# lmfaber/karma

Hardware: AMD Instinct MI355X
Metric: contigs+reads/sec for k-mer vec + shared-read graph build; HBM GB/s vs roofline (higher is better)
Workload: dtype u32 keys / i64 counts / f64 div

## Files before the change

### include/karma.h

```cpp
#ifndef KARMA_H
#define KARMA_H

#include <stddef.h>
#include <stdint.h>

#ifdef __cplusplus
extern "C" {
#endif

#define KARMA_OK 0
#define KARMA_ERR_ARG (-1)
#define KARMA_ERR_KMER (-2)
#define KARMA_ERR_HIP (-3)
#define KARMA_ERR_OOM (-4)
#define KARMA_ERR_ZERO_DIV (-5)
#define KARMA_ERR_UNSORTED (-6)
#define KARMA_ERR_STATE (-7)
#define KARMA_ERR_PARSE (-8)
#define KARMA_ERR_COMM (-9)
#define KARMA_ERR_STALL (-10)

#define KARMA_KMER_5P6 (-1)

int karma_version(void);
// ... 82 lines not shown

int karma_knn_rows(karma_ctx* ctx, const double* x, int64_t n, int64_t m, int64_t ld, int x_is_device,
                   int64_t row_lo, int64_t row_hi, int k, int32_t* idx, double* dist, int out_is_device);
int karma_knn_tile(int* query_rows, int* cand_rows, int* col_panel, int* k_max);

int karma_knn_block(karma_ctx* ctx, const double* q, int64_t nq, int64_t ldq, int q_is_device,
                    const double* c, int64_t nc, int64_t ldc, int c_is_device,
                    int64_t m, int64_t cand_base, int k,
                    uint64_t* keys, int32_t* idx, int state_is_device,
                    int first, int cand_split);
int karma_knn_merge(karma_ctx* ctx, uint64_t* keys, int32_t* idx,
                    const uint64_t* keys_b, const int32_t* idx_b,
                    int64_t nq, int k, int state_is_device);
int karma_knn_finish(karma_ctx* ctx, const uint64_t* keys, const int32_t* idx, int64_t nq, int k, int state_is_device,
                     int32_t* out_idx, double* out_dist, int out_is_device);
int karma_knn_block_split(karma_ctx* ctx, int64_t nq, int64_t nc, int cand_split, int* used);

typedef struct karma_pairs karma_pairs;
#define KARMA_REC_SORTED 0
#define KARMA_REC_UNSORTED 1
#define KARMA_REC_FLAGGED 2
int karma_graph_records(karma_ctx* ctx, const uint32_t* records, int64_t n_records, int64_t n_contigs, int flags,
                        int is_device, karma_pairs** out);
typedef struct karma_graph_job karma_graph_job;
int karma_graph_records_begin(karma_ctx* ctx, const uint32_t* records, int64_t n_records, int64_t n_contigs,
                              int flags, int is_device, karma_graph_job** job);
int karma_graph_records_end(karma_graph_job* job, karma_pairs** out);
int karma_graph_split_hint(karma_ctx* ctx, const int64_t* bounds, int nranks);
int karma_records_flag(karma_ctx* ctx, const uint32_t* records, int64_t n_records, int rec_format, int is_device,
                       uint32_t* out, int out_is_device, int64_t* n_reads);
int karma_records_flag_tile(int* per_thread, int* per_wave, int* per_block);
int karma_classify_launches(uint64_t* pairs, uint64_t* flagged);
int karma_graph_classify_occupancy(karma_ctx* ctx, int64_t n_contigs, int rec_format, int* blocks_per_cu);
int karma_graph_eq(karma_ctx* ctx, const int64_t* cls_off, const uint32_t* members, const int64_t* counts,
                   const uint8_t* pair_skip, int64_t n_classes, int64_t n_contigs, int is_device, karma_pairs** out);
int karma_graph_eq_compact(karma_ctx* ctx, const uint8_t* sizes, const uint32_t* members, int64_t n_members,
                           const uint32_t* counts, int64_t C, int64_t n_contigs, karma_pairs** out);
int karma_pairs_merge(karma_ctx* ctx, const uint64_t* keys, const int64_t* counts, int64_t n, int is_device,
                      karma_pairs** out);
int karma_pairs_merge_runs(karma_ctx* ctx, const uint64_t* keys, const int64_t* counts, const int64_t* run_off,
                           int n_runs, int is_device, karma_pairs** out);
int karma_merge_tile(int* tile, int* lds_keys, int* max_runs, int* search_group);
int karma_step_tail_tile(karma_ctx* ctx, int* v, int n);
int karma_pairs_get_kc(karma_pairs* p, int64_t* kc_dev);
int karma_pairs_merge_runs_kc(karma_ctx* ctx, const int64_t* kc_dev, const int64_t* run_off, int n_runs,
                              karma_pairs** out);
int karma_pairs_destroy(karma_pairs* p);
int karma_pairs_rebind(karma_pairs* p, karma_ctx* ctx);
int karma_pairs_count(karma_pairs* p, int64_t* n);
int karma_pairs_device(karma_pairs* p, const uint64_t** keys, const int64_t** counts);
int karma_pairs_get(karma_pairs* p, uint64_t* keys, int64_t* counts, uint64_t* first, int is_device);
int karma_pairs_split(karma_pairs* p, const int64_t* bounds, int nranks, int64_t* starts);
int karma_pairs_split_kc(karma_pairs* p, const int64_t* bounds, int nranks, int64_t* starts, int64_t* kc_dev);
int karma_pairs_totals(karma_pairs* p, int64_t* totals_dev, int64_t n_contigs);

typedef struct karma_edges karma_edges;
#define KARMA_MODE_READS 0
#define KARMA_MODE_EQ 1
int karma_edges_from_pairs(karma_ctx* ctx, karma_pairs* p, int mode, const int64_t* totals_dev, int64_t n_contigs,
                           karma_edges** out, int64_t* n_edges);
int karma_edges_begin(karma_ctx* ctx, karma_pairs* p, int mode, int64_t n_contigs, karma_edges** out,
                      int64_t** totals_dev);
int karma_edges_end(karma_edges* e, int64_t* n_edges);
int karma_edges_count(karma_edges* e, int64_t* n_edges);
int karma_edges_destroy(karma_edges* e);
int karma_edges_get(karma_edges* e, uint32_t* a, uint32_t* b, int64_t* shared, double* weight, uint64_t* first,
                    int is_device);
int karma_edges_totals(karma_edges* e, int64_t* totals, int is_device);
int karma_edges_get_all(karma_edges* e, uint32_t* a, uint32_t* b, int64_t* s, double* w, uint64_t* first,
                        int64_t* totals, int is_device);
int karma_edges_get_ordered(karma_edges* e, uint32_t* a, uint32_t* b, double* w, int is_device);

typedef struct karma_step karma_step;
#define KARMA_STEP_KEEP 1
#define KARMA_STEP_SEQUENTIAL 2
#define KARMA_STEP_FLAGGED 8
// ... 79 lines not shown
```

### karma_amd/_lib.py

```python

from __future__ import annotations

import ctypes
import os
import types
import weakref

import numpy as np

HERE = os.path.dirname(os.path.abspath(__file__))
LIB_PATH = os.environ.get("KARMA_LIB") or os.path.join(HERE, "libkarma_hip.so")

KARMA_OK = 0
KARMA_ERR_ARG = -1
KARMA_ERR_KMER = -2
KARMA_ERR_HIP = -3
KARMA_ERR_OOM = -4
KARMA_ERR_ZERO_DIV = -5
KARMA_ERR_UNSORTED = -6
KARMA_ERR_STATE = -7
KARMA_ERR_PARSE = -8
KARMA_ERR_COMM = -9
KARMA_ERR_STALL = -10

# ... 58 lines not shown
    "karma_contigs_destroy": [_c_p],
    "karma_contigs_info": [_c_p, _I64P, _I64P, _I64P, _I64P],
    "karma_kmer_plan_create": [_c_p, _c_p, _i32, _PP],
    "karma_kmer_plan_destroy": [_c_p],
    "karma_kmer_presence_words": [_c_p, _I64P],
    "karma_kmer_presence_get": [_c_p, _c_p],
    "karma_kmer_presence_set": [_c_p, _c_p],
    "karma_kmer_presence_merge": [_c_p, _c_p, _i32],
    "karma_kmer_exceptions_count": [_c_p, _I64P],
    "karma_kmer_exceptions_get": [_c_p, _c_p],
    "karma_kmer_exceptions_set": [_c_p, _c_p, _i64],
    "karma_kmer_plan_finalize": [_c_p, _I64P],
    "karma_kmer_plan_finalize_async": [_c_p],
    "karma_kmer_plan_finalize_wait": [_c_p, _I64P],
    "karma_kmer_columns": [_c_p, _c_p],
    "karma_kmer_profile": [_c_p, _c_p, _i64, _i32],
    "karma_kmer_profile_rows": [_c_p, _i64, _i64, _c_p, _i64, _i32],
    "karma_kmer_profile_side": [_c_p, _c_p, _i64, _c_p],
    "karma_ctx_join": [_c_p, _c_p],
    "karma_ctx_set_side_headroom": [_c_p, _i32],
    "karma_kmer_row_totals": [_c_p, _c_p],
    "karma_knn_rows": [_c_p, _c_p, _i64, _i64, _i64, _i32, _i64, _i64, _i32, _c_p, _c_p, _i32],
    "karma_knn_tile": [ctypes.POINTER(ctypes.c_int)] * 4,
    "karma_knn_block": [_c_p, _c_p, _i64, _i64, _i32, _c_p, _i64, _i64, _i32, _i64, _i64, _i32, _c_p, _c_p, _i32, _i32,
                        _i32],
    "karma_knn_merge": [_c_p, _c_p, _c_p, _c_p, _c_p, _i64, _i32, _i32],
    "karma_knn_finish": [_c_p, _c_p, _c_p, _i64, _i32, _i32, _c_p, _c_p, _i32],
    "karma_knn_block_split": [_c_p, _i64, _i64, _i32, ctypes.POINTER(ctypes.c_int)],
    "karma_graph_records": [_c_p, _c_p, _i64, _i64, _i32, _i32, _PP],
    "karma_graph_records_begin": [_c_p, _c_p, _i64, _i64, _i32, _i32, _PP],
    "karma_graph_records_end": [_c_p, _PP],
    "karma_graph_split_hint": [_c_p, _c_p, _i32],
    "karma_graph_classify_occupancy": [_c_p, _i64, _i32, ctypes.POINTER(ctypes.c_int)],
    "karma_records_flag": [_c_p, _c_p, _i64, _i32, _i32, _c_p, _i32, _I64P],
    "karma_records_flag_tile": [ctypes.POINTER(ctypes.c_int)] * 3,
    "karma_classify_launches": [_c_p, _c_p],
    "karma_graph_eq": [_c_p, _c_p, _c_p, _c_p, _c_p, _i64, _i64, _i32, _PP],
    "karma_graph_eq_compact": [_c_p, _c_p, _c_p, _i64, _c_p, _i64, _i64, _PP],
    "karma_pairs_merge": [_c_p, _c_p, _c_p, _i64, _i32, _PP],
    "karma_pairs_merge_runs": [_c_p, _c_p, _c_p, _c_p, _i32, _i32, _PP],
    "karma_pairs_merge_runs_kc": [_c_p, _c_p, _c_p, _i32, _PP],
    "karma_merge_tile": [ctypes.POINTER(ctypes.c_int)] * 4,
    "karma_pairs_get_kc": [_c_p, _c_p],
    "karma_pairs_destroy": [_c_p],
    "karma_pairs_rebind": [_c_p, _c_p],
    "karma_pairs_count": [_c_p, _I64P],
    "karma_pairs_device": [_c_p, _PP, _PP],
    "karma_pairs_get": [_c_p, _c_p, _c_p, _c_p, _i32],
    "karma_pairs_split": [_c_p, _c_p, _i32, _c_p],
    "karma_pairs_totals": [_c_p, _c_p, _i64],
    "karma_edges_from_pairs": [_c_p, _c_p, _i32, _c_p, _i64, _PP, _I64P],
    "karma_edges_begin": [_c_p, _c_p, _i32, _i64, _PP, _PP],
    "karma_edges_end": [_c_p, _I64P],
    "karma_edges_count": [_c_p, _I64P],
    "karma_pairs_split_kc": [_c_p, _c_p, _i32, _c_p, _c_p],
    "karma_edges_destroy": [_c_p],
    "karma_edges_get": [_c_p, _c_p, _c_p, _c_p, _c_p, _c_p, _i32],
    "karma_edges_totals": [_c_p, _c_p, _i32],
    "karma_edges_get_all": [_c_p, _c_p, _c_p, _c_p, _c_p, _c_p, _c_p, _i32],
    "karma_edges_get_ordered": [_c_p, _c_p, _c_p, _c_p, _i32],
    "karma_api_calls": [_c_p],
    "karma_step_create": [_c_p, _c_p, _c_p, _i32, _i64, _c_p, _i32, _i32, _PP],
    "karma_step_run": [_c_p, _c_p, _c_p, _i64, _i32, _c_p],
    "karma_step_sync": [_c_p],
    "karma_step_info": [_c_p, _c_p, _i32],
    "karma_step_profile": [_c_p, _PP, _I64P, _I64P],
    "karma_step_columns": [_c_p, _c_p],
    "karma_step_edges": [_c_p, _PP],
    "karma_step_newest_edges": [_c_p, _c_p, _c_p, _c_p, _c_p, _c_p, _i64, _i32, _I64P, _c_p],
    "karma_step_destroy": [_c_p],
    "karma_step_tail_tile": [_c_p, _c_p, _i32],
    "karma_synth_contig_lengths": [_u64, _i64, _i32, _i32, _c_p],
    "karma_synth_contig_bases": [_u64, _c_p, _i64, _i32, _c_p],
    "karma_synth_n_genes": [_u64, _i64, _i32, _I64P],
    "karma_synth_genes": [_u64, _i64, _i32, _c_p, _c_p],
    "karma_synth_read_counts": [_u64, _c_p, _c_p, _i64, _i64, _i64, _i32, _c_p],
    "karma_synth_read_records": [_u64, _c_p, _c_p, _i64, _i64, _i64, _i32, _c_p, _c_p],
    "karma_synth_eq_classes": [_u64, _c_p, _c_p, _i64, _i64, _i64, _i32, _I64P, _I64P, _c_p, _c_p, _c_p],
    "karma_fasta_parse": [_c_p, ctypes.c_size_t, _i32, _PP],
    "karma_fasta_info": [_c_p, _I64P, _I64P, _I64P, ctypes.POINTER(ctypes.c_int)],
    "karma_fasta_get": [_c_p, _c_p, _c_p, _c_p, _c_p, _c_p],
    "karma_fasta_view": [_c_p, _PP, _PP, _PP, _PP, _PP],
    "karma_fasta_destroy": [_c_p],
    "karma_eq_parse": [_c_p, ctypes.c_size_t, _i32, _PP],
    "karma_eq_info": [_c_p, _I64P, _I64P, _I64P, _I64P],
    "karma_eq_get": [_c_p, _c_p, _c_p, _c_p, _c_p, _c_p, _c_p],
    "karma_eq_get_compact": [_c_p, _c_p, _c_p, _c_p, _c_p, _c_p],
    "karma_eq_destroy": [_c_p],
    "karma_sam_parse": [_c_p, ctypes.c_size_t, _i32, _i32, _PP],
    "karma_sam_info": [_c_p, _I64P, _I64P, _I64P, _I64P, _I64P],
    "karma_sam_get": [_c_p, _c_p, _c_p, _c_p, _c_p, _c_p],
    "karma_sam_destroy": [_c_p],
    "karma_adj_from_edges": [_c_p, _i64, _c_p, _c_p, _c_p, _c_p, _i64, _i32, _PP],
    "karma_adj_from_lists": [_c_p, _i64, _c_p, _c_p, _c_p, _c_p, _i32, _PP],
    "karma_adj_view": [_c_p, _c_p, _i64, _PP],
    "karma_adj_keep": [_c_p, _c_p, _i64, _PP],
    "karma_adj_view_summary": [_c_p, _c_p, _i64, _c_p, _c_p, _i32, _c_p, _c_p, _c_p, _i64, _I64P,
                               ctypes.POINTER(ctypes.c_int)],
    "karma_adj_node_stats": [_c_p, _c_p, _c_p],
    "karma_adj_info": [_c_p, _I64P, _I64P],
    "karma_adj_get": [_c_p, _c_p, _c_p, _c_p, _c_p],
    "karma_adj_degrees": [_c_p, _c_p],
    "karma_adj_node_weights": [_c_p, _c_p],
    "karma_adj_edge_list": [_c_p, _c_p, _c_p, _i64, _i32, _c_p, _i64, _I64P],
# ... 250 lines not shown

def flag_tile():
    v = [ctypes.c_int(0) for _ in range(3)]
    call("karma_records_flag_tile", *[ctypes.byref(x) for x in v])
    return tuple(x.value for x in v)


def knn_tile():
    v = [ctypes.c_int(0) for _ in range(4)]
    call("karma_knn_tile", *[ctypes.byref(x) for x in v])
    return tuple(x.value for x in v)


def knn_block_split(ctx, nq, nc, cand_split=0):
    used = ctypes.c_int(0)
    call("karma_knn_block_split", ctx.h if ctx is not None else None, int(nq), int(nc), int(cand_split),
         ctypes.byref(used))
    return used.value


def merge_tile():
    v = [ctypes.c_int(0) for _ in range(4)]
    call("karma_merge_tile", *[ctypes.byref(x) for x in v])
    return tuple(x.value for x in v)


def step_tail_tile(ctx=None):
    v = np.zeros(8, np.int32)
    call("karma_step_tail_tile", ctx.h if ctx is not None else None, ptr(v), 8)
    return types.SimpleNamespace(MT=int(v[0]), MLDS=int(v[1]), MFAST=int(v[2]), MG=int(v[3]), ET=int(v[4]),
                                 MAX_RUNS=int(v[5]), merge_blocks=int(v[6]), edge_blocks=int(v[7]))


def dtype_code(dtype):
    return _DTYPE_CODE[np.dtype(dtype)]


_DEFAULT_CTX = {}


def default_context(device=0):
    ctx = _DEFAULT_CTX.get(device)
    if ctx is None:
        ctx = _DEFAULT_CTX[device] = Context(device)
    return ctx
```

### karma_amd/csrc/graph_sets.hip

```cpp

#include <algorithm>
#include <cstdlib>
#include <cstring>
#include <memory>
#include <type_traits>

#include "karma_internal.h"
#include "sets_ctrl.h"

using namespace karma;

namespace {

#include "graph_device.h"

typedef unsigned int u32x4 __attribute__((ext_vector_type(4)));

constexpr int kMaxB = 2048;
constexpr int kMaxBc = 512;
constexpr int kNarrowB = 512, kNarrowBc = 128;
constexpr int kCrSmax = 64;
constexpr int kCrPieces = 512;
constexpr int kCgShift = 18;
constexpr int kOneGroupB = 128;
// ... 1294 lines not shown
                wslot[lane] = -1;
                wave_lds_order();
                if (len && excl >= w0 && excl < w0 + 64u) wslot[excl - w0] = lane;
                wave_lds_order();
                const int rr = wave_max_incl(max(wslot[lane], carry));
                carry = __builtin_amdgcn_readlane(rr, 63);
                const int64_t off = (int64_t)(((uint64_t)(uint32_t)__shfl((int)((uint64_t)roff >> 32), rr) << 32) |
                                              (uint32_t)__shfl((int)(uint32_t)roff, rr));
                if (j < Tn) e[u] = data[off + j];
            }
#pragma unroll
            for (int u = 0; u < kWin; ++u)
                if (j0 + 64u * u + lane < Tn) count(e[u]);
        }
        if (pipe) {
            if (r0 + threads >= r_hi) break;
        } else if (__syncthreads_or(stop != nullptr && *stop != 0)) {
            return;
        }
    }
}

__device__ __forceinline__ void group_range(const unsigned* n_flush, int n_groups, int grp, int64_t* f_lo,
                                            int64_t* f_hi) {
    const int64_t nf = *n_flush;
    const int64_t per = (nf + n_groups - 1) / n_groups;
    *f_lo = min(nf, grp * per);
    *f_hi = min(nf, *f_lo + per);
}

constexpr int kCRT = 1024;
constexpr int kHistMax = 1 << (kMaxBwCompact + 2 + 3);

__global__ void __launch_bounds__(kCRT) code_reduce_kernel(const uint16_t* __restrict__ cent, RunDir dir, int Bc,
                                                           int bwc, int n_cg, uint32_t* __restrict__ part_ch) {
    __shared__ uint32_t h[kHistMax];
    __shared__ int slots[kCRT];
    const int bucket = blockIdx.x / n_cg, grp = blockIdx.x % n_cg;
    const int hn = 1 << (bwc + 3);
    for (int i = threadIdx.x; i < hn; i += kCRT) h[i] = 0;
    __syncthreads();
    int64_t f_lo, f_hi;
    group_range(dir.n, n_cg, grp, &f_lo, &f_hi);
    const int64_t R = f_hi - f_lo;
    const int S = R > 0 ? (int)max<int64_t>(1, min<int64_t>(kCrSmax, (kCrPieces + R - 1) / R)) : 1;
    auto slot = [](uint32_t c) { return c ^ ((c >> 5) & 31u); };
    auto add = [&](uint32_t c) {
        if (c != CodeStream::kPadV)
            __hip_atomic_fetch_add(&h[slot(c)], 1u, __ATOMIC_RELAXED, __HIP_MEMORY_SCOPE_WORKGROUP);
    };
    stream_runs(
        reinterpret_cast<const u32x4*>(cent), f_lo * S, f_hi * S, kCRT,
        [&](int64_t v, int64_t* beg, uint32_t* len) {
            const int64_t f = v / S;
            const uint32_t s = (uint32_t)(v - f * S);
            const uint32_t* o = dir.off + f * (Bc + 1) + bucket;
            const uint32_t L = (o[1] - o[0]) >> 3, seg = (L + S - 1) / S;
            const uint32_t lo = min(L, s * seg), hi = min(L, lo + seg);
            *beg = ((dir.base[f] + o[0]) >> 3) + lo;
            *len = hi - lo;
        },
        [&](const u32x4 v) {
            add(v.x & 0xFFFFu), add(v.x >> 16), add(v.y & 0xFFFFu), add(v.y >> 16);
            add(v.z & 0xFFFFu), add(v.z >> 16), add(v.w & 0xFFFFu), add(v.w >> 16);
        },
        nullptr, slots);
    __syncthreads();
    uint32_t* out = part_ch + (int64_t)blockIdx.x * hn;
    for (int i = threadIdx.x; i < hn; i += kCRT) out[i] = h[slot(i)];
}

__device__ __forceinline__ uint32_t nibble_sum(uint32_t x) {
    x = (x & 0x0F0F0F0Fu) + ((x >> 4) & 0x0F0F0F0Fu);
    return (x * 0x01010101u) >> 24;
}
constexpr int kBackList = 2048;
__global__ void __launch_bounds__(kCRT) code_seg_reduce_kernel(const uint16_t* __restrict__ segs,
                                                               const uint4* __restrict__ hdr,
                                                               const uint8_t* __restrict__ dir, int64_t n_chunks,
                                                               uint32_t seg_cap, int dir_cap, int bwc, int n_cg,
                                                               uint32_t* __restrict__ part_ch, uint32_t list_cap,
                                                               int slotted) {
    __shared__ uint32_t h[kHistMax];
    __shared__ int slots[kCRT];
    __shared__ uint32_t blist[kBackList];
    __shared__ uint32_t nlist;
    const int bucket = blockIdx.x / n_cg, grp = blockIdx.x % n_cg;
    const int hn = 1 << (bwc + 3);
    for (int i = threadIdx.x; i < hn; i += kCRT) h[i] = 0;
    if (threadIdx.x == 0) nlist = 0;
    __syncthreads();
    const int64_t per = (n_chunks + n_cg - 1) / n_cg;
    const int64_t c_lo = min(n_chunks, (int64_t)grp * per), c_hi = min(n_chunks, c_lo + per);
    const int wave = __builtin_amdgcn_readfirstlane(threadIdx.x >> 6), lane = threadIdx.x & 63;
    auto slot = [](uint32_t c) { return c ^ ((c >> 5) & 31u); };
    auto add = [&](uint32_t c) {
        if (c != 0xFFFFu) __hip_atomic_fetch_add(&h[slot(c)], 1u, __ATOMIC_RELAXED, __HIP_MEMORY_SCOPE_WORKGROUP);
    };
    auto add8 = [&](const u32x4 v) {
        add(v.x & 0xFFFFu), add(v.x >> 16), add(v.y & 0xFFFFu), add(v.y >> 16);
        add(v.z & 0xFFFFu), add(v.z >> 16), add(v.w & 0xFFFFu), add(v.w >> 16);
    };
    const int bw_ = bucket >> 3, bs = 4 * (bucket & 7);
    auto list_back = [&](int64_t c, uint32_t bmw) {
        if ((bmw >> (bucket & 31)) & 1u) {
            const uint32_t i = __hip_atomic_fetch_add(&nlist, 1u, __ATOMIC_RELAXED, __HIP_MEMORY_SCOPE_WORKGROUP);
            if (i < list_cap) blist[i] = (uint32_t)(c - c_lo);
        }
    };
    if (slotted) {
        const uint32_t* const hw = reinterpret_cast<const uint32_t*>(hdr + 2) + (bucket < 32 ? 0 : 1);
        const uint32_t loff = (uint32_t)(lane >> 3) * seg_cap * (kBinQ * 2) + 16u * (lane & 7);
        const uint32_t tstr = 8u * seg_cap * (kBinQ * 2);
        auto load = [&](u32x4 (&v)[8], uint32_t& bm, int64_t c0, auto whole) {
            const char* const p = reinterpret_cast<const char*>(segs + (c0 * seg_cap + bucket) * kBinQ);
#pragma unroll
            for (int t = 0; t < 8; ++t)
                if (whole || c0 + 8 * t + (lane >> 3) < c_hi)
                    v[t] = *reinterpret_cast<const u32x4*>(p + (loff + t * tstr));
            if (whole || c0 + lane < c_hi) bm = hw[4 * kBinHdr * (c0 + lane)];
        };
        auto count = [&](const u32x4 (&v)[8], uint32_t bm, int64_t c0, auto whole) {
// ... 78 lines not shown
        uint64_t mb = lanes((bm >> bucket) & 1ull);
        if (!mb) continue;
        const uint32_t nb = h1.w;
        const uint32_t d[4] = {h2.z, h2.w, h3.x, h3.y};
        uint32_t hit = 0;
#pragma unroll
        for (int k = 0; k < 16; ++k)
            hit |= (((d[k >> 2] >> (8 * (k & 3))) & 0xFFu) == bb && (uint32_t)k < nb) ? 1u << k : 0u;
        for (uint32_t base = 0;;) {
            for (;;) {
                const uint64_t mm = lanes(in_mask(mb) && hit != 0u);
                if (!mm) break;
                uint32_t sg = 0;
                if (hit) {
                    const uint32_t k = (uint32_t)__builtin_ctz(hit);
                    hit &= hit - 1u;
                    sg = (uint32_t)c * seg_cap + seg_cap - 1u - (base + k);
                }
                stream8(mm, sg);
            }
            base += 16;
            mb &= lanes(base < nb);
            if (!mb) break;
            if (in_mask(mb)) {
                const u32x4 q = *reinterpret_cast<const u32x4*>(dir + c * (int64_t)dir_cap + base);
                const uint32_t e[4] = {q.x, q.y, q.z, q.w};
#pragma unroll
                for (int k = 0; k < 16; ++k)
                    hit |= (((e[k >> 2] >> (8 * (k & 3))) & 0xFFu) == bb && base + k < nb) ? 1u << k : 0u;
            }
        }
    }
    __syncthreads();
    uint32_t* out = part_ch + (int64_t)blockIdx.x * hn;
    for (int i = threadIdx.x; i < hn; i += kCRT) out[i] = h[slot(i)];
}

constexpr int kRT = 1024;
constexpr int kBand = 8192;
constexpr int kHashR = 4096;
constexpr int kHashF = 8192;
constexpr int kFT = 512;
constexpr int kSlotCap = kBand + kHashF;

template <int CAP, int THREADS>
struct HTab {
    uint32_t* keys;
    uint32_t* vals;
    int* nuniq;
    __device__ void init() {
        for (int t = threadIdx.x; t < CAP; t += THREADS) {
            keys[t] = kEmpty;
            vals[t] = 0;
        }
        if (threadIdx.x == 0) *nuniq = 0;
    }
    __device__ __forceinline__ bool insert(uint32_t key, uint32_t c) {
        uint32_t h = hash32(key) & (CAP - 1);
        for (int probe = 0; probe < CAP; ++probe) {
            const uint32_t k = __hip_atomic_load(&keys[h], __ATOMIC_RELAXED, __HIP_MEMORY_SCOPE_WORKGROUP);
            if (k == key) {
                atomicAdd(&vals[h], c);
                return true;
            }
            if (k == kEmpty) {
                const uint32_t old = atomicCAS(&keys[h], kEmpty, key);
                if (old == kEmpty || old == key) {
                    if (old == kEmpty) atomicAdd(nuniq, 1);
// ... 1165 lines not shown

void sets_release(SetsJob* job) {
    if (!job) return;
    job->ctx->job_open = false;
    job->ctx->mark_set = false;
    delete job;
}

int records_to_pairs_sets(karma_ctx* ctx, RecIn rec, int64_t A, int64_t N, karma_pairs* out) {
    if (N > kMaxCompactN) return records_to_pairs_wide(ctx, rec, A, N, out);
    SetsJob* job = nullptr;
    KARMA_TRY(sets_begin(ctx, rec, A, N, SetsOpts{}, &job));
    return sets_end(job, out);
}

}

extern "C" int karma_graph_classify_occupancy(karma_ctx* ctx, int64_t n_contigs, int rec_format,
                                              int* blocks_per_cu) {
    using namespace karma;
    KARMA_CHECK(ctx && blocks_per_cu && n_contigs >= 1 && n_contigs <= kMaxCompactN, KARMA_ERR_ARG,
                "karma_graph_classify_occupancy: bad arguments (n_contigs %lld)", (long long)n_contigs);
    KARMA_TRY(ctx_begin(ctx));
    Geo g{};
    KARMA_TRY(make_geo(n_contigs, &g));
    const bool bin = class_binned(g.Bc);
    const size_t lds = bin ? class_bin_lds(g.Bc) : 0;
    return with_classify(rec_format == KARMA_REC_FLAGGED, g.Bc >= kAppendMinBc, bin, false, [&](auto kern) -> int {
        KARMA_HIP(hipOccupancyMaxActiveBlocksPerMultiprocessor(blocks_per_cu, reinterpret_cast<const void*>(kern),
                                                               kCW, lds));
        return KARMA_OK;
    });
}
```

### karma_amd/csrc/step.hip

```cpp
#include <algorithm>
#include <chrono>
#include <cstdlib>
#include <cstring>
#include <deque>
#include <initializer_list>
#include <memory>
#include <thread>
#include <vector>

#include "karma_internal.h"
#include "sets_ctrl.h"
#include "step_schedule.h"

using namespace karma;

namespace {

constexpr int kRing = 64;
constexpr int kLag = 3;

enum StepErr : int64_t { kErrOrder = 1, kErrRange = 2, kErrPartition = 4, kErrZeroTotal = 8, kErrMergeOrder = 16 };
struct StepStatus {
    uint64_t seq;
    int64_t slow;
    int64_t err;
    int64_t U;
    int64_t E;
    int64_t pad[3];
};
static_assert(sizeof(StepStatus) == 64, "status entry");

constexpr int kET = 512;
constexpr int kMaxRuns = 64;

__device__ __forceinline__ bool is_head(const uint64_t* __restrict__ k, int64_t i, uint64_t key) {
    return i == 0 || k[i - 1] != key;
}
__device__ __forceinline__ int64_t run_sum(const uint64_t* __restrict__ k, const int64_t* __restrict__ c, int64_t n,
                                           int64_t i, uint64_t key) {
    int64_t s = c[i];
    for (int64_t j = i + 1; j < n && k[j] == key; ++j) s += c[j];
    return s;
}

__global__ void __launch_bounds__(kET) step_edge_count_kernel(const uint64_t* __restrict__ keys,
                                                              const int64_t* __restrict__ counts,
                                                              const int64_t* __restrict__ n_dev, int64_t n_tot,
                                                              int64_t* __restrict__ totals,
                                                              int64_t* __restrict__ tile_cnt,
                                                              int64_t* __restrict__ st) {
    const int64_t n = *n_dev;
    if (blockIdx.x == 0 && threadIdx.x < 3) st[threadIdx.x] = 0;
    const int64_t stride = (int64_t)gridDim.x * kET, gid = (int64_t)blockIdx.x * kET + threadIdx.x;
    const int64_t a_first = n ? (int64_t)(keys[0] >> 32) : n_tot;
    const int64_t a_last = n ? (int64_t)(keys[n - 1] >> 32) : n_tot;
    for (int64_t c = gid; c < min(a_first, n_tot); c += stride) totals[c] = 0;
    for (int64_t c = a_last + 1 + gid; c < n_tot; c += stride) totals[c] = 0;
    const int64_t tiles = (n + kET - 1) / kET;
    for (int64_t t = blockIdx.x; t < tiles; t += gridDim.x) {
        const int64_t i = t * kET + threadIdx.x;
        bool f = false;
        if (i < n) {
            const uint64_t k = keys[i];
            const uint32_t a = (uint32_t)(k >> 32), b = (uint32_t)k;
            if (i > 0) {
                const uint32_t pa = (uint32_t)(keys[i - 1] >> 32);
                const uint32_t lim = (int64_t)a < n_tot ? a : (uint32_t)n_tot;
                for (uint32_t c = pa + 1; c < lim; ++c) totals[c] = 0;
                if ((int64_t)a < n_tot && pa != a && a != b) totals[a] = 0;
            } else if ((int64_t)a < n_tot && a != b) {
                totals[a] = 0;
            }
            if (is_head(keys, i, k) && (int64_t)b < n_tot) {
                const int64_t s = run_sum(keys, counts, n, i, k);
                if (a == b) totals[a] = s;
                else f = s != 0;
            }
        }
        const int cnt = __syncthreads_count(f);
        if (threadIdx.x == 0) tile_cnt[t] = cnt;
    }
}

__global__ void __launch_bounds__(kET) step_edge_write_kernel(
    const uint64_t* __restrict__ keys, const int64_t* __restrict__ counts, const int64_t* __restrict__ n_dev,
    const int64_t* __restrict__ totals, const int64_t* __restrict__ tile_cnt, uint32_t* __restrict__ ea,
    uint32_t* __restrict__ eb, int64_t* __restrict__ es, double* __restrict__ ew, int64_t* __restrict__ st,
    int64_t n_tot) {
    __shared__ int64_t wsum[kET / 64];
    __shared__ int64_t base_s;
    const int64_t n = *n_dev;
    const int64_t tiles = (n + kET - 1) / kET;
    const int lane = threadIdx.x & 63, wave = threadIdx.x >> 6;
    if (blockIdx.x == 0 && tiles == 0 && threadIdx.x == 0) st[2] = 0;
    for (int64_t t = blockIdx.x; t < tiles; t += gridDim.x) {
        int64_t b = 0;
        for (int64_t j = threadIdx.x; j < t; j += kET) b += tile_cnt[j];
#pragma unroll
        for (int d = 32; d >= 1; d >>= 1) b += __shfl_xor(b, d, 64);
        if (lane == 0) wsum[wave] = b;
        __syncthreads();
        if (threadIdx.x == 0) {
            int64_t s = 0;
            for (int w = 0; w < kET / 64; ++w) s += wsum[w];
            base_s = s;
        }
        const int64_t i = t * kET + threadIdx.x;
        uint64_t k = 0;
        int64_t c = 0;
        bool f = false;
        if (i < n) {
            k = keys[i];
            const uint32_t a = (uint32_t)(k >> 32), bb = (uint32_t)k;
            if ((int64_t)bb >= n_tot) {
                st[1] = 1;
            } else if (a != bb && is_head(keys, i, k)) {
                c = run_sum(keys, counts, n, i, k);
                f = c != 0;
            }
        }
        const uint64_t m = __ballot(f);
        __syncthreads();
        if (lane == 0) wsum[wave] = __popcll(m);
        __syncthreads();
        int64_t before = 0, total = 0;
        for (int w = 0; w < kET / 64; ++w) {
            if (w < wave) before += wsum[w];
            total += wsum[w];
        }
        const int64_t base = base_s;
        if (t == tiles - 1 && threadIdx.x == 0) st[2] = base + total;
        if (f) {
            const int64_t o = base + before + __popcll(m & ((1ull << lane) - 1ull));
            const uint32_t a = (uint32_t)(k >> 32), bb = (uint32_t)k;
            const int64_t ta = totals[a], tb = totals[bb];
            ea[o] = a;
            eb[o] = bb;
            es[o] = c;
            if (ta == 0 || tb == 0) {
                st[0] = 1;
                ew[o] = 0.0;
            } else {
                const double x = __ddiv_rn((double)c, (double)ta);
                const double y = __ddiv_rn((double)c, (double)tb);
                ew[o] = __dadd_rn(x, y) * 0.5;
            }
        }
        __syncthreads();
    }
}

constexpr int kMT = 1024;
constexpr int kMLds = 8192;
constexpr int kMFast = 8;
constexpr int kMG = 16;
constexpr int kMergePerCu = 8, kEdgePerCu = 4;
struct RunSrc {
    int nr, B, bw;
    int64_t b[kMaxRuns + 1];
    int64_t slot = 0;
    int64_t* n_out = nullptr;
};

__device__ __forceinline__ int64_t count_below(const uint64_t* __restrict__ a, int64_t lo, int64_t hi, uint64_t k,
                                               bool le) {
    int64_t n = hi - lo, base = lo;
    while (n > 0) {
        const int64_t half = n >> 1;
        const uint64_t m = a[base + half];
        const bool before = le ? m <= k : m < k;
        base = before ? base + half + 1 : base;
        n = before ? n - half - 1 : half;
    }
    return base;
}

__global__ void __launch_bounds__(256) step_merge_kernel(const uint64_t* __restrict__ keys,
                                                         const int64_t* __restrict__ counts,
                                                         const int64_t* __restrict__ dst,
                                                         const int64_t* __restrict__ split_loc, RunSrc rs,
                                                         uint64_t* __restrict__ ko, int64_t* __restrict__ co,
                                                         int64_t* __restrict__ bad) {
    __shared__ int64_t ro[kMaxRuns + 1], re[kMaxRuns + 1], rt[kMaxRuns + 1];
    __shared__ int64_t wlo[kMaxRuns], whi[kMaxRuns];
    __shared__ int wbase[kMaxRuns];
    __shared__ int all_fit;
    __shared__ uint64_t wkeys[kMLds];
    const int nr = rs.nr;
    const int64_t U = rs.slot > 0 ? 0 : dst[rs.B];
// ... 805 lines not shown
        const int64_t* mcounts = v.counts;
        if (s->world > 1) {
            const int W = s->world;
            const int64_t slot = s->kc + 1;
            KARMA_TRY(ensure_arr(ctx, tl.sk, W * slot));
            KARMA_TRY(ensure_arr(ctx, tl.sc, W * slot));
            KARMA_TRY(ensure_arr(ctx, tl.rk, W * slot));
            KARMA_TRY(ensure_arr(ctx, tl.rc, W * slot));
            KARMA_TRY(ensure_arr(ctx, tl.nm, 1));
            KARMA_LAUNCH(ctx, "exchange_pack", step_pack_kernel,
                         (int)std::max<int64_t>(1, std::min<int64_t>((v.cap + 255) / 256, 4 * cu)), 256, 0, v.keys,
                         v.counts, v.dst, v.split_loc, rs, slot, tl.sk.ptr, tl.sc.ptr, v.flags, v.counters, v.ovf);
            std::vector<int64_t> off(W + 1);
            for (int r = 0; r <= W; ++r) off[r] = (int64_t)r * slot * 8;
            KARMA_TRY(karma_comm_alltoallv_kv(s->comm, tl.sk.ptr, tl.sc.ptr, off.data(), tl.rk.ptr, tl.rc.ptr,
                                              off.data()));
            rs.slot = slot;
            rs.n_out = tl.nm.ptr;
            mkeys = tl.rk.ptr;
            mcounts = tl.rc.ptr;
            cap = W * (slot - 1);
            n_dev = tl.nm.ptr;
        }
        KARMA_TRY(ensure_arr(ctx, tl.mk, cap));
        KARMA_TRY(ensure_arr(ctx, tl.mc, cap));
        const int64_t tiles_cap = (cap + kMT - 1) / kMT + s->nranks;
        KARMA_LAUNCH(ctx, "merge_rank", step_merge_kernel, (int)std::min<int64_t>(tiles_cap, kMergePerCu * cu), 256, 0,
                     mkeys, mcounts, v.dst, v.split_loc, rs, tl.mk.ptr, tl.mc.ptr, tl.mbad.ptr);
        lk = tl.mk.ptr;
        lc = tl.mc.ptr;
        mbad = tl.mbad.ptr;
    }
    KARMA_TRY(ensure_arr(ctx, tl.tot, s->n_glob));
    KARMA_TRY(ensure_arr(ctx, tl.tile_cnt, (cap + kET - 1) / kET + 1));
    KARMA_TRY(ensure_arr(ctx, tl.est, 3));
    KARMA_TRY(ensure_arr(ctx, tl.ea, cap));
    KARMA_TRY(ensure_arr(ctx, tl.eb, cap));
    KARMA_TRY(ensure_arr(ctx, tl.es, cap));
    KARMA_TRY(ensure_arr(ctx, tl.ew, cap));
    const int grid = (int)std::max<int64_t>(1, std::min<int64_t>((cap + kET - 1) / kET, kEdgePerCu * cu));
    KARMA_LAUNCH(ctx, "edge_count", step_edge_count_kernel, grid, kET, 0, lk, lc, n_dev, s->n_glob, tl.tot.ptr,
                 tl.tile_cnt.ptr, tl.est.ptr);
    if (s->world > 1) KARMA_TRY(allgather_slices(s, tl.tot.ptr));
    KARMA_LAUNCH(ctx, "edge_weights", step_edge_write_kernel, grid, kET, 0, lk, lc, n_dev, tl.tot.ptr,
                 tl.tile_cnt.ptr, tl.ea.ptr, tl.eb.ptr, tl.es.ptr, tl.ew.ptr, tl.est.ptr, s->n_glob);
    KARMA_CHECK(seq != s->fault_seq, KARMA_ERR_STATE, "karma_step: injected fault in deferred step %llu",
                (unsigned long long)seq);
    KARMA_LAUNCH(ctx, "step_status", step_status_kernel, 1, 256, 0, v.flags, v.counters, v.ovf, v.B, v.dst, mbad,
                 tl.est.ptr, s->ring_d + seq % kRing, seq, v.ctrl, v.ctrl ? v.ctrl_need : (int64_t)0);
    if (sc.xs_on) {
        if (!s->ev_tail[sc.par]) KARMA_HIP(hipEventCreateWithFlags(&s->ev_tail[sc.par], hipEventDisableTiming));
        KARMA_HIP(hipEventRecord(s->ev_tail[sc.par], q.xs));
        s->tail_set[sc.par] = true;
        s->tail_last = sc.par;
    }
    return KARMA_OK;
}

struct FailGuard {
    karma_step* s;
    karma_step::Tail& tl;
    uint64_t seq;
    bool armed = true;
    ~FailGuard() {
        if (!armed) return;
        (void)sync_all({s->side_s, s->side_alt_s, s->main_s, s->alt_s}, true);
        if (tl.ctrl.ptr) {
            (void)hipMemsetAsync(tl.ctrl.ptr, 0, tl.ctrl.n * 8, s->main_s);
            (void)hipStreamSynchronize(s->main_s);
        }
        if (s->prof_seq == seq) {
            s->prof_seq = 0;
            s->prof_M = -1;
        }
    }
};

// ... 209 lines not shown
        if (is_device) KARMA_TRY(karma_ctx_sync(s->ctx));
        return KARMA_OK;
    }
    const karma_step::Tail& tl = s->tail[s->prof_par];
    const int64_t E = const_cast<const StepStatus&>(s->ring_h[s->prof_seq % kRing]).E;
    KARMA_CHECK(E >= 0 && E <= (int64_t)tl.ea.n, KARMA_ERR_STATE, "karma_step_newest_edges: bad edge count %lld",
                (long long)E);
    *n_edges = E;
    if (deferred) *deferred = 1;
    if ((a || b || shared || weight) && E > cap) {
        set_error("karma_step_newest_edges: %lld edges, room for %lld", (long long)E, (long long)cap);
        return KARMA_ERR_ARG;
    }
    hipStream_t q = s->main_s;
    if (E) {
        if (a) KARMA_HIP(hipMemcpyAsync(a, tl.ea.ptr, E * 4, kind, q));
        if (b) KARMA_HIP(hipMemcpyAsync(b, tl.eb.ptr, E * 4, kind, q));
        if (shared) KARMA_HIP(hipMemcpyAsync(shared, tl.es.ptr, E * 8, kind, q));
        if (weight) KARMA_HIP(hipMemcpyAsync(weight, tl.ew.ptr, E * 8, kind, q));
    }
    if (totals) KARMA_HIP(hipMemcpyAsync(totals, tl.tot.ptr, s->n_glob * 8, kind, q));
    KARMA_HIP(hipStreamSynchronize(q));
    return KARMA_OK;
}

int karma_step_tail_tile(karma_ctx* ctx, int* v, int n) {
    KARMA_CHECK(v && n >= 0, KARMA_ERR_ARG, "karma_step_tail_tile: bad arguments");
    const int cu = ctx ? ctx->cu_count : 0;
    const int c[] = {kMT, kMLds, kMFast, kMG, kET, kMaxRuns, kMergePerCu * cu, kEdgePerCu * cu};
    for (int i = 0; i < n && i < (int)(sizeof c / sizeof c[0]); ++i) v[i] = c[i];
    return KARMA_OK;
}

int karma_step_destroy(karma_step* s) {
    if (!s) return KARMA_OK;
    hipSetDevice(s->ctx->device);
    (void)sync_all({s->main_s, s->alt_s, s->side_s, s->side_alt_s}, true);
    s->pending.clear();
    s->E = 0;
    drop_outputs(s);
    bury(s, true);
    for (auto& ev : s->grave_ev)
        if (ev) hipEventDestroy(ev);
    for (hipEvent_t ev : {s->ev_rec, s->ev_sync, s->ev_tail[0], s->ev_tail[1], s->ev_pres, s->ev_pres2, s->ev_pre,
                          s->ev_passed})
        if (ev) hipEventDestroy(ev);
    if (s->graves_h) hipHostFree(s->graves_h);
    if (s->ring_mem) hipHostFree(s->ring_mem);
    s->prof.release();
    s->m_ring.release();
    s->plan_zero[0].release();
    s->plan_zero[1].release();
    for (auto& tl : s->tail) tl.release();
    karma_ctx* ctx = s->ctx;
    hipStream_t prev = ctx->stream;
    if (prev == s->main_s || prev == s->side_s || prev == s->alt_s || prev == s->side_alt_s)
        ctx->stream = ctx->own_stream;
    if (s->side_alt_s) karma_stream_destroy(ctx, s->side_alt_s);
    if (s->side_s) karma_stream_destroy(ctx, s->side_s);
    if (s->alt_s) karma_stream_destroy(ctx, s->alt_s);
    if (s->main_s) karma_stream_destroy(ctx, s->main_s);
    delete s;
    return KARMA_OK;
}

}
// ... 1 lines not shown
```

Baseline: 131.8 billion.

## Prefetch next edge tile and merge block syncs in edge write kernel

```diff
diff --git a/include/karma.h b/include/karma.h
--- a/include/karma.h
+++ b/include/karma.h
@@ -138,6 +138,8 @@
 int karma_records_flag_tile(int* per_thread, int* per_wave, int* per_block);
 int karma_classify_launches(uint64_t* pairs, uint64_t* flagged);
 int karma_graph_classify_occupancy(karma_ctx* ctx, int64_t n_contigs, int rec_format, int* blocks_per_cu);
+int karma_graph_code_hist(karma_ctx* ctx, const uint16_t* codes, int64_t n_codes, int bwc, int layout,
+                          uint32_t* part_ch);
 int karma_graph_eq(karma_ctx* ctx, const int64_t* cls_off, const uint32_t* members, const int64_t* counts,
                    const uint8_t* pair_skip, int64_t n_classes, int64_t n_contigs, int is_device, karma_pairs** out);
 int karma_graph_eq_compact(karma_ctx* ctx, const uint8_t* sizes, const uint32_t* members, int64_t n_members,
@@ -148,6 +150,9 @@
                            int n_runs, int is_device, karma_pairs** out);
 int karma_merge_tile(int* tile, int* lds_keys, int* max_runs, int* search_group);
 int karma_step_tail_tile(karma_ctx* ctx, int* v, int n);
+int karma_step_edge_stage(karma_ctx* ctx, const uint64_t* keys, const int64_t* counts, int64_t n, int64_t cap,
+                          int64_t n_glob, int64_t* totals, int64_t* tile_cnt, int64_t* st, uint32_t* ea,
+                          uint32_t* eb, int64_t* es, double* ew);
 int karma_pairs_get_kc(karma_pairs* p, int64_t* kc_dev);
 int karma_pairs_merge_runs_kc(karma_ctx* ctx, const int64_t* kc_dev, const int64_t* run_off, int n_runs,
                               karma_pairs** out);
diff --git a/karma_amd/_lib.py b/karma_amd/_lib.py
--- a/karma_amd/_lib.py
+++ b/karma_amd/_lib.py
@@ -114,6 +114,7 @@
     "karma_graph_records_end": [_c_p, _PP],
     "karma_graph_split_hint": [_c_p, _c_p, _i32],
     "karma_graph_classify_occupancy": [_c_p, _i64, _i32, ctypes.POINTER(ctypes.c_int)],
+    "karma_graph_code_hist": [_c_p, _c_p, _i64, _i32, _i32, _c_p],
     "karma_records_flag": [_c_p, _c_p, _i64, _i32, _i32, _c_p, _i32, _I64P],
     "karma_records_flag_tile": [ctypes.POINTER(ctypes.c_int)] * 3,
     "karma_classify_launches": [_c_p, _c_p],
@@ -152,6 +153,7 @@
     "karma_step_newest_edges": [_c_p, _c_p, _c_p, _c_p, _c_p, _c_p, _i64, _i32, _I64P, _c_p],
     "karma_step_destroy": [_c_p],
     "karma_step_tail_tile": [_c_p, _c_p, _i32],
+    "karma_step_edge_stage": [_c_p, _c_p, _c_p, _i64, _i64, _i64, _c_p, _c_p, _c_p, _c_p, _c_p, _c_p, _c_p],
     "karma_synth_contig_lengths": [_u64, _i64, _i32, _i32, _c_p],
     "karma_synth_contig_bases": [_u64, _c_p, _i64, _i32, _c_p],
     "karma_synth_n_genes": [_u64, _i64, _i32, _I64P],
@@ -468,6 +470,28 @@
                                  MAX_RUNS=int(v[5]), merge_blocks=int(v[6]), edge_blocks=int(v[7]))
 
 
+def step_edge_stage(ctx, keys, counts, cap, n_glob):
+    keys = np.ascontiguousarray(keys, np.uint64)
+    counts = np.ascontiguousarray(counts, np.int64)
+    n, et = len(keys), step_tail_tile().ET
+    assert len(counts) == n
+    r = types.SimpleNamespace(totals=np.empty(n_glob, np.int64), tile_cnt=np.empty(-(-cap // et) + 1, np.int64),
+                              st=np.empty(3, np.int64), a=np.empty(cap, np.uint32), b=np.empty(cap, np.uint32),
+                              shared=np.empty(cap, np.int64), weight=np.empty(cap, np.float64))
+    call("karma_step_edge_stage", ctx.h, ptr(keys), ptr(counts), n, cap, n_glob, ptr(r.totals), ptr(r.tile_cnt),
+         ptr(r.st), ptr(r.a), ptr(r.b), ptr(r.shared), ptr(r.weight))
+    return r
+
+
+def graph_code_hist(ctx, codes, bwc, layout):
+    codes = np.asarray(codes, np.uint16)
+    padded = np.full(-(-len(codes) // 64) * 64, 0xFFFF, np.uint16)
+    padded[:len(codes)] = codes
+    out = np.empty(8 << bwc, np.uint32)
+    call("karma_graph_code_hist", ctx.h, ptr(padded), len(padded), bwc, layout, ptr(out))
+    return out
+
+
 def dtype_code(dtype):
     return _DTYPE_CODE[np.dtype(dtype)]
 
diff --git a/karma_amd/csrc/graph_sets.hip b/karma_amd/csrc/graph_sets.hip
--- a/karma_amd/csrc/graph_sets.hip
+++ b/karma_amd/csrc/graph_sets.hip
@@ -1350,13 +1350,25 @@
 constexpr int kCRT = 1024;
 constexpr int kHistMax = 1 << (kMaxBwCompact + 2 + 3);
 
+__device__ __forceinline__ void hist_clear(uint32_t* h, int hn) {
+    for (int i = 4 * threadIdx.x; i < hn; i += 4 * kCRT) *reinterpret_cast<u32x4*>(h + i) = u32x4{0u, 0u, 0u, 0u};
+}
+__device__ __forceinline__ void hist_write_out(const uint32_t* h, int hn, uint32_t* __restrict__ out) {
+    for (int i = 4 * threadIdx.x; i < hn; i += 4 * kCRT) {
+        const uint32_t x = ((uint32_t)i >> 5) & 31u;
+        const u32x4 v = *reinterpret_cast<const u32x4*>(h + ((uint32_t)i ^ (x & ~3u)));
+        const u32x4 s = (x & 1u) ? u32x4{v.y, v.x, v.w, v.z} : v;
+        *reinterpret_cast<u32x4*>(out + i) = (x & 2u) ? u32x4{s.z, s.w, s.x, s.y} : s;
+    }
+}
+
 __global__ void __launch_bounds__(kCRT) code_reduce_kernel(const uint16_t* __restrict__ cent, RunDir dir, int Bc,
                                                            int bwc, int n_cg, uint32_t* __restrict__ part_ch) {
-    __shared__ uint32_t h[kHistMax];
+    __shared__ __attribute__((aligned(16))) uint32_t h[kHistMax];
     __shared__ int slots[kCRT];
     const int bucket = blockIdx.x / n_cg, grp = blockIdx.x % n_cg;
     const int hn = 1 << (bwc + 3);
-    for (int i = threadIdx.x; i < hn; i += kCRT) h[i] = 0;
+    hist_clear(h, hn);
     __syncthreads();
     int64_t f_lo, f_hi;
     group_range(dir.n, n_cg, grp, &f_lo, &f_hi);
@@ -1384,8 +1396,7 @@
         },
         nullptr, slots);
     __syncthreads();
-    uint32_t* out = part_ch + (int64_t)blockIdx.x * hn;
-    for (int i = threadIdx.x; i < hn; i += kCRT) out[i] = h[slot(i)];
+    hist_write_out(h, hn, part_ch + (int64_t)blockIdx.x * hn);
 }
 
 __device__ __forceinline__ uint32_t nibble_sum(uint32_t x) {
@@ -1399,13 +1410,13 @@
                                                                uint32_t seg_cap, int dir_cap, int bwc, int n_cg,
                                                                uint32_t* __restrict__ part_ch, uint32_t list_cap,
                                                                int slotted) {
-    __shared__ uint32_t h[kHistMax];
+    __shared__ __attribute__((aligned(16))) uint32_t h[kHistMax];
     __shared__ int slots[kCRT];
     __shared__ uint32_t blist[kBackList];
     __shared__ uint32_t nlist;
     const int bucket = blockIdx.x / n_cg, grp = blockIdx.x % n_cg;
     const int hn = 1 << (bwc + 3);
-    for (int i = threadIdx.x; i < hn; i += kCRT) h[i] = 0;
+    hist_clear(h, hn);
     if (threadIdx.x == 0) nlist = 0;
     __syncthreads();
     const int64_t per = (n_chunks + n_cg - 1) / n_cg;
@@ -1550,8 +1561,7 @@
         }
     }
     __syncthreads();
-    uint32_t* out = part_ch + (int64_t)blockIdx.x * hn;
-    for (int i = threadIdx.x; i < hn; i += kCRT) out[i] = h[slot(i)];
+    hist_write_out(h, hn, part_ch + (int64_t)blockIdx.x * hn);
 }
 
 constexpr int kRT = 1024;
@@ -2783,3 +2793,50 @@
         return KARMA_OK;
     });
 }
+
+extern "C" int karma_graph_code_hist(karma_ctx* ctx, const uint16_t* codes, int64_t n_codes, int bwc, int layout,
+                                     uint32_t* part_ch) {
+    using namespace karma;
+    KARMA_CHECK(ctx && part_ch && (codes || !n_codes) && n_codes >= 0 && n_codes % kBinQ == 0 &&
+                    n_codes < (int64_t(1) << 30) && bwc >= 0 && bwc <= kMaxBwCompact + 2 && layout >= 0 && layout <= 2,
+                KARMA_ERR_ARG, "karma_graph_code_hist: bad arguments");
+    KARMA_TRY(ctx_begin(ctx));
+    const int64_t hn = int64_t(8) << bwc, n_chunks = n_codes / kBinQ;
+    DevArray<uint16_t> d;
+    DevArray<uint32_t> out, hdr, off;
+    DevArray<uint8_t> dir;
+    DevArray<int64_t> base;
+    DevArray<unsigned> nf;
+    KARMA_TRY(d.alloc(ctx, n_codes));
+    KARMA_TRY(out.alloc(ctx, hn));
+    hipStream_t q = ctx->stream;
+    if (n_codes) KARMA_HIP(hipMemcpyAsync(d.ptr, codes, n_codes * 2, hipMemcpyHostToDevice, q));
+    KARMA_HIP(hipMemsetAsync(out.ptr, 0xA5, hn * 4, q));
+    if (layout == 0) {
+        const int64_t b0 = 0;
+        const uint32_t o[2] = {0u, (uint32_t)n_codes};
+        const unsigned one = 1;
+        KARMA_TRY(base.alloc(ctx, 1));
+        KARMA_TRY(off.alloc(ctx, 2));
+        KARMA_TRY(nf.alloc(ctx, 1));
+        KARMA_HIP(hipMemcpyAsync(base.ptr, &b0, 8, hipMemcpyHostToDevice, q));
+        KARMA_HIP(hipMemcpyAsync(off.ptr, o, 8, hipMemcpyHostToDevice, q));
+        KARMA_HIP(hipMemcpyAsync(nf.ptr, &one, 4, hipMemcpyHostToDevice, q));
+        KARMA_HIP(hipStreamSynchronize(q));
+        const RunDir rd{base.ptr, off.ptr, nf.ptr, nullptr};
+        KARMA_LAUNCH(ctx, "graph_code_reduce", code_reduce_kernel, 1, kCRT, 0, d.ptr, rd, 1, bwc, 1, out.ptr);
+    } else {
+        std::vector<uint32_t> h((size_t)n_chunks * kBinHdr * 4, 0u);
+        for (int64_t c = 0; c < n_chunks; ++c) h[(size_t)c * kBinHdr * 4] = kBinQ / 8;
+        KARMA_TRY(hdr.alloc(ctx, h.size()));
+        KARMA_TRY(dir.alloc(ctx, 16));
+        if (n_chunks) KARMA_HIP(hipMemcpyAsync(hdr.ptr, h.data(), h.size() * 4, hipMemcpyHostToDevice, q));
+        KARMA_HIP(hipStreamSynchronize(q));
+        KARMA_LAUNCH(ctx, "graph_code_reduce", code_seg_reduce_kernel, 1, kCRT, 0, d.ptr,
+                     reinterpret_cast<const uint4*>(hdr.ptr), dir.ptr, n_chunks, 1u, 16, bwc, 1, out.ptr,
+                     (uint32_t)kBackList, layout == 1 ? 1 : 0);
+    }
+    KARMA_HIP(hipMemcpyAsync(part_ch, out.ptr, hn * 4, hipMemcpyDeviceToHost, q));
+    KARMA_HIP(hipStreamSynchronize(q));
+    return KARMA_OK;
+}
diff --git a/karma_amd/csrc/step.hip b/karma_amd/csrc/step.hip
--- a/karma_amd/csrc/step.hip
+++ b/karma_amd/csrc/step.hip
@@ -32,6 +32,33 @@
 
 constexpr int kET = 512;
 constexpr int kMaxRuns = 64;
+
+struct EdgeElem {
+    uint64_t kp, k, kn;
+    int64_t c, cn;
+};
+__device__ __forceinline__ EdgeElem edge_elem_load(const uint64_t* __restrict__ keys,
+                                                   const int64_t* __restrict__ counts, int64_t i, int64_t cap) {
+    const int64_t hi = cap - 1;
+    const int64_t ic = min(i, hi), ip = max(ic - 1, (int64_t)0), in = min(i + 1, hi);
+    EdgeElem e;
+    e.kp = keys[ip];
+    e.k = keys[ic];
+    e.kn = keys[in];
+    e.c = counts[ic];
+    e.cn = counts[in];
+    return e;
+}
+__device__ __forceinline__ bool is_head(const EdgeElem& e, int64_t i) { return i == 0 || e.kp != e.k; }
+__device__ __forceinline__ int64_t run_sum(const uint64_t* __restrict__ k, const int64_t* __restrict__ c, int64_t n,
+                                           int64_t i, const EdgeElem& e) {
+    int64_t s = e.c;
+    if (i + 1 < n && e.kn == e.k) {
+        s += e.cn;
+        for (int64_t j = i + 2; j < n && k[j] == e.k; ++j) s += c[j];
+    }
+    return s;
+}
 
 __device__ __forceinline__ bool is_head(const uint64_t* __restrict__ k, int64_t i, uint64_t key) {
     return i == 0 || k[i - 1] != key;
@@ -82,58 +109,76 @@
     }
 }
 
+__host__ __device__ constexpr int64_t edge_tile_cap(int64_t cap) { return (cap + kET - 1) / kET + 1; }
+
+struct EdgeTileIn {
+    EdgeElem e;
+    int64_t p0, p1;
+};
+__device__ __forceinline__ EdgeTileIn edge_tile_load(const uint64_t* __restrict__ keys,
+                                                     const int64_t* __restrict__ counts,
+                                                     const int64_t* __restrict__ tile_cnt, int64_t t, int64_t cap) {
+    const int64_t tc_hi = edge_tile_cap(cap) - 1;
+    EdgeTileIn in;
+    in.e = edge_elem_load(keys, counts, t * kET + threadIdx.x, cap);
+    in.p0 = tile_cnt[min((int64_t)threadIdx.x, tc_hi)];
+    in.p1 = tile_cnt[min((int64_t)threadIdx.x + kET, tc_hi)];
+    return in;
+}
+
 __global__ void __launch_bounds__(kET) step_edge_write_kernel(
     const uint64_t* __restrict__ keys, const int64_t* __restrict__ counts, const int64_t* __restrict__ n_dev,
-    const int64_t* __restrict__ totals, const int64_t* __restrict__ tile_cnt, uint32_t* __restrict__ ea,
-    uint32_t* __restrict__ eb, int64_t* __restrict__ es, double* __restrict__ ew, int64_t* __restrict__ st,
-    int64_t n_tot) {
-    __shared__ int64_t wsum[kET / 64];
-    __shared__ int64_t base_s;
+    int64_t cap, const int64_t* __restrict__ totals, const int64_t* __restrict__ tile_cnt,
+    uint32_t* __restrict__ ea, uint32_t* __restrict__ eb, int64_t* __restrict__ es, double* __restrict__ ew,
+    int64_t* __restrict__ st, int64_t n_tot) {
+    __shared__ int64_t wpre[kET / 64];
+    __shared__ int wcnt[kET / 64];
+    const int lane = threadIdx.x & 63, wave = threadIdx.x >> 6;
+    EdgeTileIn in = edge_tile_load(keys, counts, tile_cnt, blockIdx.x, cap);
     const int64_t n = *n_dev;
     const int64_t tiles = (n + kET - 1) / kET;
-    const int lane = threadIdx.x & 63, wave = threadIdx.x >> 6;
     if (blockIdx.x == 0 && tiles == 0 && threadIdx.x == 0) st[2] = 0;
-    for (int64_t t = blockIdx.x; t < tiles; t += gridDim.x) {
-        int64_t b = 0;
-        for (int64_t j = threadIdx.x; j < t; j += kET) b += tile_cnt[j];
+    auto tile = [&](const EdgeTileIn& ti, int64_t t) {
+        const EdgeElem& e = ti.e;
+        const int64_t i = t * kET + threadIdx.x;
+        const uint32_t a = (uint32_t)(e.k >> 32), bb = (uint32_t)e.k;
+        const bool in_range = i < n && (int64_t)bb < n_tot;
+        const bool pair = in_range && a != bb && (int64_t)a < n_tot;
+        int64_t b = ((int64_t)threadIdx.x < t ? ti.p0 : 0) + ((int64_t)threadIdx.x + kET < t ? ti.p1 : 0);
+        for (int64_t j = (int64_t)threadIdx.x + 2 * kET; j < t; j += kET) b += tile_cnt[j];
+        int64_t ta = 0, tb = 0;
+        if (pair) {
+            ta = totals[a];
+            tb = totals[bb];
+        }
+        int64_t c = 0;
+        bool f = false;
+        if (i < n && !in_range) {
+            st[1] = 1;
+        } else if (pair && is_head(e, i)) {
+            c = run_sum(keys, counts, n, i, e);
+            f = c != 0;
+        }
 #pragma unroll
         for (int d = 32; d >= 1; d >>= 1) b += __shfl_xor(b, d, 64);
-        if (lane == 0) wsum[wave] = b;
+        const uint64_t m = __ballot(f);
+        if (lane == 0) {
+            wpre[wave] = b;
+            wcnt[wave] = __popcll(m);
+        }
         __syncthreads();
-        if (threadIdx.x == 0) {
-            int64_t s = 0;
-            for (int w = 0; w < kET / 64; ++w) s += wsum[w];
-            base_s = s;
-        }
-        const int64_t i = t * kET + threadIdx.x;
-        uint64_t k = 0;
-        int64_t c = 0;
-        bool f = false;
-        if (i < n) {
-            k = keys[i];
-            const uint32_t a = (uint32_t)(k >> 32), bb = (uint32_t)k;
-            if ((int64_t)bb >= n_tot) {
-                st[1] = 1;
-            } else if (a != bb && is_head(keys, i, k)) {
-                c = run_sum(keys, counts, n, i, k);
-                f = c != 0;
-            }
-        }
-        const uint64_t m = __ballot(f);
-        __syncthreads();
-        if (lane == 0) wsum[wave] = __popcll(m);
-        __syncthreads();
-        int64_t before = 0, total = 0;
+        int64_t base = 0;
+        int before = 0, total = 0;
+#pragma unroll
         for (int w = 0; w < kET / 64; ++w) {
-            if (w < wave) before += wsum[w];
-            total += wsum[w];
-        }
-        const int64_t base = base_s;
+            base += wpre[w];
+            const int x = wcnt[w];
+            before += w < wave ? x : 0;
+            total += x;
+        }
         if (t == tiles - 1 && threadIdx.x == 0) st[2] = base + total;
         if (f) {
             const int64_t o = base + before + __popcll(m & ((1ull << lane) - 1ull));
-            const uint32_t a = (uint32_t)(k >> 32), bb = (uint32_t)k;
-            const int64_t ta = totals[a], tb = totals[bb];
             ea[o] = a;
             eb[o] = bb;
             es[o] = c;
@@ -147,6 +192,17 @@
             }
         }
         __syncthreads();
+    };
+    for (int64_t t = blockIdx.x; t < tiles;) {
+        const int64_t tn = t + gridDim.x;
+        if (tn < tiles) {
+            const EdgeTileIn nx = edge_tile_load(keys, counts, tile_cnt, tn, cap);
+            tile(in, t);
+            in = nx;
+        } else {
+            tile(in, t);
+        }
+        t = tn;
     }
 }
 
@@ -155,6 +211,9 @@
 constexpr int kMFast = 8;
 constexpr int kMG = 16;
 constexpr int kMergePerCu = 8, kEdgePerCu = 4;
+inline int edge_grid(int64_t cap, int cu) {
+    return (int)std::max<int64_t>(1, std::min<int64_t>((cap + kET - 1) / kET, (int64_t)kEdgePerCu * cu));
+}
 struct RunSrc {
     int nr, B, bw;
     int64_t b[kMaxRuns + 1];
@@ -1026,17 +1085,18 @@
         mbad = tl.mbad.ptr;
     }
     KARMA_TRY(ensure_arr(ctx, tl.tot, s->n_glob));
-    KARMA_TRY(ensure_arr(ctx, tl.tile_cnt, (cap + kET - 1) / kET + 1));
+    KARMA_CHECK(cap >= 1, KARMA_ERR_STATE, "karma_step: an edge stage without list capacity");
+    KARMA_TRY(ensure_arr(ctx, tl.tile_cnt, edge_tile_cap(cap)));
     KARMA_TRY(ensure_arr(ctx, tl.est, 3));
     KARMA_TRY(ensure_arr(ctx, tl.ea, cap));
     KARMA_TRY(ensure_arr(ctx, tl.eb, cap));
     KARMA_TRY(ensure_arr(ctx, tl.es, cap));
     KARMA_TRY(ensure_arr(ctx, tl.ew, cap));
-    const int grid = (int)std::max<int64_t>(1, std::min<int64_t>((cap + kET - 1) / kET, kEdgePerCu * cu));
+    const int grid = edge_grid(cap, cu);
     KARMA_LAUNCH(ctx, "edge_count", step_edge_count_kernel, grid, kET, 0, lk, lc, n_dev, s->n_glob, tl.tot.ptr,
                  tl.tile_cnt.ptr, tl.est.ptr);
     if (s->world > 1) KARMA_TRY(allgather_slices(s, tl.tot.ptr));
-    KARMA_LAUNCH(ctx, "edge_weights", step_edge_write_kernel, grid, kET, 0, lk, lc, n_dev, tl.tot.ptr,
+    KARMA_LAUNCH(ctx, "edge_weights", step_edge_write_kernel, grid, kET, 0, lk, lc, n_dev, cap, tl.tot.ptr,
                  tl.tile_cnt.ptr, tl.ea.ptr, tl.eb.ptr, tl.es.ptr, tl.ew.ptr, tl.est.ptr, s->n_glob);
     KARMA_CHECK(seq != s->fault_seq, KARMA_ERR_STATE, "karma_step: injected fault in deferred step %llu",
                 (unsigned long long)seq);
@@ -1312,6 +1372,60 @@
     return KARMA_OK;
 }
 
+int karma_step_edge_stage(karma_ctx* ctx, const uint64_t* keys, const int64_t* counts, int64_t n, int64_t cap,
+                          int64_t n_glob, int64_t* totals, int64_t* tile_cnt, int64_t* st, uint32_t* ea,
+                          uint32_t* eb, int64_t* es, double* ew) {
+    KARMA_CHECK(ctx && totals && tile_cnt && st && ea && eb && es && ew, KARMA_ERR_ARG,
+                "karma_step_edge_stage: null argument");
+    KARMA_CHECK(cap >= 1 && n >= 0 && n <= cap && n_glob >= 1 && (!n || (keys && counts)), KARMA_ERR_ARG,
+                "karma_step_edge_stage: bad sizes");
+    KARMA_HIP(hipSetDevice(ctx->device));
+    DevArray<uint64_t> dk;
+    DevArray<int64_t> dc, dn, dtot, dtc, dst, des;
+    DevArray<uint32_t> dea, deb;
+    DevArray<double> dew;
+    const int64_t tc = edge_tile_cap(cap);
+    KARMA_TRY(dk.alloc(ctx, cap));
+    KARMA_TRY(dc.alloc(ctx, cap));
+    KARMA_TRY(dn.alloc(ctx, 1));
+    KARMA_TRY(dtot.alloc(ctx, n_glob));
+    KARMA_TRY(dtc.alloc(ctx, tc));
+    KARMA_TRY(dst.alloc(ctx, 3));
+    KARMA_TRY(dea.alloc(ctx, cap));
+    KARMA_TRY(deb.alloc(ctx, cap));
+    KARMA_TRY(des.alloc(ctx, cap));
+    KARMA_TRY(dew.alloc(ctx, cap));
+    hipStream_t q = ctx->stream;
+    KARMA_HIP(hipMemsetAsync(dk.ptr, 0xA5, cap * 8, q));
+    KARMA_HIP(hipMemsetAsync(dc.ptr, 0xA5, cap * 8, q));
+    if (n) {
+        KARMA_HIP(hipMemcpyAsync(dk.ptr, keys, n * 8, hipMemcpyHostToDevice, q));
+        KARMA_HIP(hipMemcpyAsync(dc.ptr, counts, n * 8, hipMemcpyHostToDevice, q));
+    }
+    KARMA_HIP(hipMemcpyAsync(dn.ptr, &n, 8, hipMemcpyHostToDevice, q));
+    KARMA_HIP(hipMemsetAsync(dtot.ptr, 0xA5, n_glob * 8, q));
+    KARMA_HIP(hipMemsetAsync(dtc.ptr, 0xA5, tc * 8, q));
+    KARMA_HIP(hipMemsetAsync(dst.ptr, 0xA5, 3 * 8, q));
+    KARMA_HIP(hipMemsetAsync(dea.ptr, 0xA5, cap * 4, q));
+    KARMA_HIP(hipMemsetAsync(deb.ptr, 0xA5, cap * 4, q));
+    KARMA_HIP(hipMemsetAsync(des.ptr, 0xA5, cap * 8, q));
+    KARMA_HIP(hipMemsetAsync(dew.ptr, 0xA5, cap * 8, q));
+    const int grid = edge_grid(cap, ctx->cu_count);
+    KARMA_LAUNCH(ctx, "edge_count", step_edge_count_kernel, grid, kET, 0, dk.ptr, dc.ptr, dn.ptr, n_glob, dtot.ptr,
+                 dtc.ptr, dst.ptr);
+    KARMA_LAUNCH(ctx, "edge_weights", step_edge_write_kernel, grid, kET, 0, dk.ptr, dc.ptr, dn.ptr, cap, dtot.ptr,
+                 dtc.ptr, dea.ptr, deb.ptr, des.ptr, dew.ptr, dst.ptr, n_glob);
+    KARMA_HIP(hipMemcpyAsync(totals, dtot.ptr, n_glob * 8, hipMemcpyDeviceToHost, q));
+    KARMA_HIP(hipMemcpyAsync(tile_cnt, dtc.ptr, tc * 8, hipMemcpyDeviceToHost, q));
+    KARMA_HIP(hipMemcpyAsync(st, dst.ptr, 3 * 8, hipMemcpyDeviceToHost, q));
+    KARMA_HIP(hipMemcpyAsync(ea, dea.ptr, cap * 4, hipMemcpyDeviceToHost, q));
+    KARMA_HIP(hipMemcpyAsync(eb, deb.ptr, cap * 4, hipMemcpyDeviceToHost, q));
+    KARMA_HIP(hipMemcpyAsync(es, des.ptr, cap * 8, hipMemcpyDeviceToHost, q));
+    KARMA_HIP(hipMemcpyAsync(ew, dew.ptr, cap * 8, hipMemcpyDeviceToHost, q));
+    KARMA_HIP(hipStreamSynchronize(q));
+    return KARMA_OK;
+}
+
 int karma_step_destroy(karma_step* s) {
     if (!s) return KARMA_OK;
     hipSetDevice(s->ctx->device);
```

After: 131.4 billion. Within noise of the previous version (-0.3%).
